# fanzhongyi/diffusion

Measured on AMD Instinct MI355X. Metric: U-Net training images/sec @256 (SD-2-base U-Net, precomputed latents 4x32x32), higher is better.
Workload: dtype bf16; 1 GPU; SD-2-base U-Net train step, latents 4x32x32, text 77x1024, batch 256/GPU (global 256), microbatch 256, AdamW, dp1; global_batch=256, microbatch=256, parallelism=dp1, params=865910724

## Files before the change

diffusion_amd/csrc/gemm_nt.hip:

```cpp
#include <string.h>

#include "common.hpp"
#include "diffusion_amd.h"

namespace {

struct GemmNTParams {
  const bf16* A;
  const bf16* W;
  void* C;
  const float* bias;
  const bf16* rowbias;
  const bf16* R;
  long lda, ldc, ldrb, ldr;
  int M, N, K, Cin;
  int Hin, Win, Hout, Wout;
  int ksize, mode;
  int out_fp32;
  float alpha;
  int tiles_m, tiles_n;
};

constexpr int BM = 128, BN = 128, BK = 64;
constexpr int STAGE_BYTES = (BM + BN) * BK * 2;
// ... 199 lines not shown

int da_gemm_nt_v2_dispatch(int variant, int splits, float* ws, const void* A, long lda, const void* W, void* C, long ldc, const float* bias,
                           const void* rowbias, long ldrb, const void* R, long ldr, int M, int N, int K, int Cin,
                           int Hin, int Win, int Hout, int Wout, int ksize, int mode, int out_fp32, float alpha,
                           hipStream_t stream);

int da_gemm_nt_v3_try(const void* A, long lda, const void* W, void* C, long ldc, const float* bias, const void* R, long ldr,
                      int M, int N, int K, hipStream_t stream);
extern int g_nt_stream, g_nt_stream_lw;
int da_gemm_nt_ws_try(const void* A, long lda, const void* W, const float* bias, const void* R, long ldr, void* C, long ldc,
                      int M, int N, int K, hipStream_t stream);
extern int g_nt_ws;

extern int g_tn_variant;
extern int g_nt_korder;
extern int g_nt_persist;
extern int g_reserve_cus;
extern int g_nt_persist_conv;
extern int g_nt_de;
extern int g_grad_overwrite;
extern int g_attn_fused_bwd;
extern int g_tn_ring, g_tn_ungroup;
extern int g_gn_resident, g_gn_resident_form, g_gn_resident_min_slab;
int da_usable_cus(int cus);
static int g_nt_variant = 0;
static int g_nt_mfma32 = 0;
static int g_nt_splitk = 1;

static int g_nt_dispatch = 1;

// ... 6 lines not shown
  if (N % 160 != 0 && tm * ((N + 127) / 128) >= 200) return 4;
  if (N % 320 == 0 && g_nt_splitk) {
    const long tiles = tm * (N / 320);
    const int nk = K / 64;
    int s = (int)((256 + tiles - 1) / tiles);
    if (s > 8) s = 8;
    while (s > 1 && (nk / s < 8 || (long)s * M * N > ws_floats)) --s;
    if (s > 1 && tiles * s >= 96) {
      *splits = s;
      return 12;
    }
  }
  return 1;
}

static int pick_nt_variant(int M, int N, int K, int Cin, long ws_floats, int* splits) {
  *splits = 1;
  if (Cin % 64 != 0) return 1;
  if (g_nt_variant == 4 || g_nt_variant == 5 || g_nt_variant == 10 || g_nt_variant == 11 || g_nt_variant == 12 || g_nt_variant == 14 ||
      g_nt_variant == 15 || g_nt_variant == 16 || g_nt_variant == 18)
    return g_nt_variant;
  if (g_nt_variant != 0) return 1;
  if (!g_nt_dispatch) return pick_nt_variant_legacy(M, N, K, Cin, ws_floats, splits);
  struct Form { int variant, bm, bn; double step_us, fixed_us; };
  static const Form forms[] = {{12, 256, 320, 1.5, 8.0}, {14, 256, 256, 1.3, 8.0}, {5, 256, 160, 1.16, 6.0}, {18, 384, 128, 1.37, 8.0},
                               {4, 256, 128, 1.07, 5.0}};
  const int nk = K / 64;
  const int ncu = da_usable_cus(256);
  double best = 1e30;
  int best_v = 4, best_s = 1;
  for (const Form& f : forms) {
    const long tiles = ((M + f.bm - 1) / f.bm) * ((N + f.bn - 1) / f.bn);
    for (int s = 1; s <= (g_nt_splitk ? 8 : 1); ++s) {
      if (s > 1 && (nk / s < 4 || (long)s * M * N > ws_floats)) break;
      const long rounds = (tiles * s + ncu - 1) / ncu;
      const int steps = (nk + s - 1) / s;
      double t = (double)rounds * (steps * f.step_us + f.fixed_us);
      if (s > 1) t += 20.0 + ((double)s * M * N * 4.0 + (double)M * N * 2.0) / 5.0e6;
      if (t < best * 0.97) {
        best = t;
        best_v = f.variant;
        best_s = s;
      }
    }
  }
  *splits = best_s;
  if (best_v == 12 && (g_nt_mfma32 == 1 || (g_nt_mfma32 < 0 && K <= 320))) return 15;
  return best_v;
}

extern "C" int da_gemm_nt_variant_for(int M, int N, int K, int Cin, long ws_floats) {
  int s;
// ... 3 lines not shown
extern "C" int da_set_option(const char* key, int value) {
  if (key && !strcmp(key, "gemm_nt_variant")) {
    g_nt_variant = value;
    return DA_OK;
  }
  if (key && !strcmp(key, "gemm_nt_splitk")) {
    g_nt_splitk = value;
    return DA_OK;
  }
  if (key && !strcmp(key, "gemm_nt_dispatch")) {
    g_nt_dispatch = value;
    return DA_OK;
  }
  if (key && !strcmp(key, "gemm_nt_persist")) {
    g_nt_persist = value;
    return DA_OK;
  }
  if (key && !strcmp(key, "gemm_nt_korder")) {
    g_nt_korder = value;
    return DA_OK;
  }
  if (key && !strcmp(key, "gemm_nt_mfma32")) {
    g_nt_mfma32 = value;
    return DA_OK;
  }
  if (key && !strcmp(key, "gemm_tn_variant")) {
    g_tn_variant = value;
    return DA_OK;
  }
  if (key && !strcmp(key, "attn_fused_bwd")) {
// ... 71 lines not shown
  if (mode == 4 && ksize != 3) return DA_ERR_SHAPE;
  if (Hout <= 0 || Wout <= 0 || (M % (Hout * Wout))) return DA_ERR_SHAPE;
  if (R && (ldr & 7)) return DA_ERR_SHAPE;
  if (rowbias && (ldrb & 7)) return DA_ERR_SHAPE;
  if (g_nt_ws && g_nt_variant == 0 && ksize == 1 && mode == 0 && !out_fp32 && alpha == 1.0f && !rowbias) {
    const int rc = da_gemm_nt_ws_try(A, lda, W, bias, R, ldr, C, ldc, M, N, K, stream);
    if (rc >= 0) return rc;
  }
  if (g_nt_stream && g_nt_variant == 0 && ksize == 1 && mode == 0 && !out_fp32 && alpha == 1.0f && !rowbias &&
      (g_nt_stream == 2 || (K <= 640 && (long)((M + 127) / 128) * ((N + 319) / 320) >= 512))) {
    const int rc = da_gemm_nt_v3_try(A, lda, W, C, ldc, bias, R, ldr, M, N, K, stream);
    if (rc >= 0) return rc;
  }
  {
    int splits = 1;
    const int variant = pick_nt_variant(M, N, K, Cin, splitk_ws ? splitk_ws_floats : 0, &splits);
    if (variant != 1)
      return da_gemm_nt_v2_dispatch(variant, splits, splitk_ws, A, lda, W, C, ldc, bias, rowbias, ldrb, R, ldr, M, N, K, Cin, Hin, Win,
                                    Hout, Wout, ksize, mode, out_fp32, alpha, stream);
  }
  GemmNTParams p;
  p.A = (const bf16*)A; p.W = (const bf16*)W; p.C = C; p.bias = bias;
  p.rowbias = (const bf16*)rowbias; p.R = (const bf16*)R;
  p.lda = lda; p.ldc = ldc; p.ldrb = ldrb; p.ldr = ldr;
  p.M = M; p.N = N; p.K = K; p.Cin = Cin;
  p.Hin = Hin; p.Win = Win; p.Hout = Hout; p.Wout = Wout;
  p.ksize = ksize; p.mode = mode; p.out_fp32 = out_fp32; p.alpha = alpha;
  p.tiles_m = (M + BM - 1) / BM;
  p.tiles_n = (N + BN - 1) / BN;
  static unsigned long long attr_done = 0;
  if (da_ensure_dyn_smem((const void*)gemm_nt_kernel, SMEM_BYTES, &attr_done) != DA_OK) return DA_ERR_LAUNCH;
// ... 5 lines not shown
```

diffusion_amd/csrc/gemm_nt_v2.hip:

```cpp
#include "common.hpp"
#include "diffusion_amd.h"
#ifndef NT2_NT
#define NT2_NT 0
#endif
#if NT2_NT
#define NTST st8_nt
#else
#define NTST st8
#endif


#ifndef NT2_CT
#define NT2_CT 1
#endif

int g_nt_persist = -1;
int g_reserve_cus = 0;
int g_nt_persist_conv = 1;
int g_nt_de = 1;
int da_usable_cus(int cus) {
  int n = cus - g_reserve_cus;
  return n < 32 ? 32 : n;
}

namespace {

struct GemmNT2Params {
  const bf16* A;
  const bf16* W;
  void* C;
  const float* bias;
  const bf16* rowbias;
  const bf16* R;
  long lda, ldc, ldrb, ldr;
  int M, N, K, Cin;
  int Hin, Win, Hout, Wout;
  int ksize, mode;
  int out_fp32;
  float alpha;
  int tiles_m, tiles_n;
  int splits, ksteps_per_split;
  long slab_stride;
  bf16* G;
  long ldg;
  int inner;
  int total_blocks;
  FastDiv div_hw, div_w;
  FastDiv div_nblk, div_tn;
  int korder;
};

__device__ __attribute__((aligned(256))) unsigned char g_zero_page[256];

template <int BK>
DEVINL int swz_key(int row) { return BK == 64 ? ((row >> 1) & 7) : ((row >> 2) & 3); }
template <int BK>
DEVINL int swz2(int row, int chunk) { return row * (BK * 2) + ((chunk ^ swz_key<BK>(row)) << 4); }

DEVINL void lds_barrier() {
  asm volatile("s_waitcnt lgkmcnt(0)" ::: "memory");
  __builtin_amdgcn_s_barrier();
  asm volatile("" ::: "memory");
}

// ... 4 lines not shown
    if (threadIdx.x == 0 && g_stamp_buf) g_stamp_buf[(long)vblock * 16 + (i)] = __builtin_amdgcn_s_memtime(); \
  } while (0)
extern "C" int da_debug_set_stamps(void* buf) {
  return hipMemcpyToSymbol(HIP_SYMBOL(g_stamp_buf), &buf, sizeof(buf)) == hipSuccess ? 0 : -1;
}
#else
#define STAMP(i) do {} while (0)
#endif

DEVINL void glds16(const void* gsrc, char* lds_dst) {
  __builtin_amdgcn_global_load_lds((const __attribute__((address_space(1))) void*)gsrc,
                                   (__attribute__((address_space(3))) void*)lds_dst, 16, 0, 0);
}

template <int MT, int NT, int WM, int WN, int BK, bool UPS, int GEGLU, bool EARLY, int MF = 16, bool PERSIST = EARLY, bool DE = false,
          bool HASR = false>
DEVINL void nt2_tile(const GemmNT2Params& p, const int vblock0, char* smem) {
  constexpr int NW = WM * WN;
  constexpr bool CT = MF == 16 && GEGLU == 0 && ((NT2_CT && !EARLY) || DE);
  static_assert(!DE || (MF == 16 && GEGLU == 0 && ((NT % 2) == 0 || (MT % 2) == 0)), "direct epilogue: 16x16 tiles in pairs");
  constexpr int V2_BM = MF * MT * WM, V2_BK = BK;
  static_assert((NW == 16 || NW == 8 || NW == 4) && (BK == 64 || BK == 32), "wave grid");
  static_assert(MF == 16 || (MF == 32 && GEGLU == 0 && BK == 64), "MFMA shape");
  constexpr int BN = MF * NT * WN;
  constexpr int SR = MF == 16 ? 16 : 8;
  constexpr int RG = 512 / BK;
  constexpr int LR = BK / 8;
  constexpr int AJ = V2_BM / RG / NW;
  constexpr int BGROUPS = BN / RG;
  constexpr int BJ = (BGROUPS + NW - 1) / NW;
  constexpr int A_BYTES = V2_BM * V2_BK * 2;
  constexpr int B_BYTES = BN * V2_BK * 2;
  constexpr int STAGE = A_BYTES + B_BYTES;
// ... 9 lines not shown
  const int wm = wave / WN, wn = wave % WN;
  auto task_of = [&](int ln, int pss, int tasks) {
    const bool ragged_last = (tasks % (64 * WN)) != 0 && pss == (tasks + 64 * WN - 1) / (64 * WN) - 1;
    const int slot = ragged_last ? (wn + WN - (wm * WN / 4) % WN) % WN : wn;
    return slot * 64 + ln + 64 * WN * pss;
  };
  auto fresh_lane = [&]() {
    int ln = lane;
    asm volatile("" : "+v"(ln));
    return ln;
  };
  STAMP(0);

  const int nblk = p.tiles_m * p.tiles_n;
  int split, tn, m0, n0;
  auto locate = [&](int vb) {
    split = (PERSIST && !EARLY) ? (int)fdiv((unsigned)vb, p.div_nblk) : vb / nblk;
    int bid = vb - split * nblk;
    const int q = nblk >> 3, r = nblk & 7;
    const int xcd = bid & 7, idx = bid >> 3;
    bid = (xcd < r ? xcd * (q + 1) : r * (q + 1) + (xcd - r) * q) + idx;
    const int tm = (PERSIST && !EARLY) ? (int)fdiv((unsigned)bid, p.div_tn) : bid / p.tiles_n;
    tn = bid - tm * p.tiles_n;
    m0 = tm * V2_BM;
    n0 = tn * BN;
  };
  auto wrow = [&](int c) {
    if constexpr (GEGLU == 1) return c < BN / 2 ? tn * (BN / 2) + c : p.inner + tn * (BN / 2) + (c - BN / 2);
    else return n0 + c;
  };
  const int HWo = p.Hout * p.Wout;
  constexpr bool PCONV = PERSIST && !EARLY;
  const int pad = PCONV ? 1 : ((p.ksize == 3 && p.mode != 4) ? 1 : 0);
  const int gmul = PCONV ? 1 : ((p.mode == 1 || p.mode == 4) ? 2 : 1), gshift = PCONV ? 0 : ((p.mode == 2 || p.mode == 3) ? 1 : 0),
            pmask = PCONV ? 0 : ((p.mode == 2) ? 1 : 0);
  const int hlim = gshift ? 2 * p.Hin : p.Hin, wlim = gshift ? 2 * p.Win : p.Win;
  const char* zero = reinterpret_cast<const char*>(g_zero_page);
  auto load_bias = [&](int buf) {
    if (tid < BN / 4) {
      const int n = wrow(tid * 4);
      const void* src = (p.bias && n < p.N) ? (const void*)(p.bias + n) : (const void*)zero;
      glds16(src, smem + BIAS_OFF + buf * (BN * 4) + wave * 1024);
    }
  };

  const int ntaps = PCONV ? 9 : p.ksize * p.ksize;
  const bf16* abase[AJ];
  unsigned amask[AJ];
  unsigned aoff[AJ];
  unsigned woff[BJ];
  int nk, tap, c0;
  const int nk_total = p.K / V2_BK;
  const bool tap_inner = p.korder != 0 && ntaps > 1;
  auto describe = [&]() {
  const int dl = fresh_lane();
  const int lrow = dl / LR, lchunk = dl % LR;
#pragma unroll
  for (int j = 0; j < AJ; ++j) {
    const int row = (wave * AJ + j) * RG + lrow;
    const int m = m0 + row;
    const bool mval = m < p.M;
    if constexpr (EARLY) {
#ifdef NT2_EXP_AHOT
      aoff[j] = (unsigned)(row) * (unsigned)(p.lda * 2) + (lchunk ^ swz_key<BK>(row)) * 16;
#else
      aoff[j] = (unsigned)(mval ? m : 0) * (unsigned)(p.lda * 2) + (lchunk ^ swz_key<BK>(row)) * 16;
#endif
      continue;
    }
    const int mm = mval ? m : 0;
    int b, rem, oh;
    if constexpr (PERSIST) {
      b = (int)fdiv((unsigned)mm, p.div_hw);
      rem = mm - b * HWo;
      oh = (int)fdiv((unsigned)rem, p.div_w);
    } else {
      b = mm / HWo;
      rem = mm - b * HWo;
      oh = rem / p.Wout;
    }
    const int ow = rem - oh * p.Wout;
    unsigned mask = ((oh & 1) << 16) | ((ow & 1) << 17);
    for (int t = 0; t < ntaps; ++t) {
      const int r = (PCONV || p.ksize == 3) ? t / 3 : 0, s2 = (PCONV || p.ksize == 3) ? t - 3 * r : 0;
      const int th = oh * gmul + r - pad, tw = ow * gmul + s2 - pad;
      const bool ok = mval && (unsigned)th < (unsigned)hlim && (unsigned)tw < (unsigned)wlim && !((th | tw) & pmask);
      mask |= (ok ? 1u : 0u) << t;
    }
    const int bh = (oh * gmul - pad) >> gshift, bw = (ow * gmul - pad) >> gshift;
    if constexpr (PERSIST && !UPS) {
      aoff[j] = (unsigned)(((long)(b * p.Hin * p.Win) + (long)bh * p.Win + bw) * p.lda * 2 + (lchunk ^ swz_key<BK>(row)) * 16);
      if (j == 0) amask[0] = mask & 0x1ffu;
      else amask[0] |= (mask & 0x1ffu) << (9 * j);
      continue;
    }
    amask[j] = mask;
    abase[j] = p.A + ((long)(b * p.Hin * p.Win) + (long)bh * p.Win + bw) * p.lda + (lchunk ^ swz_key<BK>(row)) * 8;
  }
#pragma unroll
  for (int j = 0; j < BJ; ++j) {
    const int g = wave + NW * j;
    const int row = g * RG + lrow;
    const int n = min(wrow(row), p.N - 1);
    woff[j] = ((unsigned)n * (unsigned)p.K + (lchunk ^ swz_key<BK>(row)) * 8) * 2;
  }

  const int kstep_begin = split * p.ksteps_per_split;
  nk = min(p.ksteps_per_split, nk_total - kstep_begin);
  if (tap_inner) {
    const int ch = kstep_begin / ntaps;
    tap = kstep_begin - ch * ntaps;
    c0 = ch * V2_BK;
  } else {
    const int kb = kstep_begin * V2_BK;
    tap = kb / p.Cin;
    c0 = kb - tap * p.Cin;
  }
  };
  auto issue = [&](int stage, bool live) {
    char* Ab = smem + stage * STAGE;
    char* Bb = Ab + A_BYTES;
    const int r = tap / 3, s2 = tap - 3 * r;
    const unsigned tapbit = live ? (1u << tap) : 0u;
// ... 30 lines not shown
        glds16(src, Ab + (wave * AJ + j) * 1024);
      }
    }
    const char* wb = reinterpret_cast<const char*>(p.W + (live ? tap * p.Cin + c0 : 0));
#pragma unroll
    for (int j = 0; j < BJ; ++j) {
      const int g = wave + NW * j;
      if constexpr (PERSIST && !EARLY) {
        if (BGROUPS % NW == 0 || g < BGROUPS) glds16(wb + (size_t)j * (NW * RG) * p.K * 2 + woff[0], Bb + g * 1024);
      } else {
        if (BGROUPS % NW == 0 || g < BGROUPS) glds16(wb + woff[j], Bb + g * 1024);
      }
    }
    const int tap_n = tap + 1, c_n = c0 + V2_BK;
    const bool wrap_t = tap_n >= ntaps, wrap_c = c_n >= p.Cin;
    if (tap_inner) {
      tap = wrap_t ? 0 : tap_n;
      c0 = wrap_t ? c_n : c0;
    } else {
      c0 = wrap_c ? 0 : c_n;
      tap = wrap_c ? tap_n : tap;
    }
  };

  typedef float accv_t __attribute__((ext_vector_type(MF == 16 ? 4 : 16)));
  accv_t acc[MT][NT];

  auto compute_half = [&](int stage, int s) {
    const char* Ab = smem + stage * STAGE;
    const char* Bb = Ab + A_BYTES;
    bf16x8 a[MT], b[NT];
// ... 81 lines not shown
      KSTAMP(2);
    } else {
      issue((t + 1) & 1, t + 1 < nk);
      compute_half(t & 1, 0);
    }
    __syncthreads();
    KSTAMP(3);
  }
#ifdef DA_STAMPS
  if (threadIdx.x == 0 && g_stamp_buf)
    for (int i = 0; i < 4; ++i) g_stamp_buf[(long)vblock * 16 + 8 + i] = ph[i];
#endif
  STAMP(3);
  };

  auto epilogue = [&](const int m0e, const int n0e, const int tne, const int splite, const int bbuf) {
  if constexpr (DE) {
    typedef unsigned u32x2_t __attribute__((ext_vector_type(2)));
    constexpr int NPJ = NT / 2;
    constexpr bool ODD = (NT & 1) != 0;
    constexpr int IH = ODD ? ((MT / 2 + 1) / 2) * 2 : (MT + 1) / 2;
    const int ln = fresh_lane();
    char* const cb = reinterpret_cast<char*>(p.C);
    const char* const rb = reinterpret_cast<const char*>(p.R);
    const int lrow = wm * (16 * MT) + (ln & 15), lq = (ln >> 4) & 1, lcol = wn * (16 * NT) + 8 * (ln >> 5);
    auto row_of = [&](int i) { return m0e + lrow + i * 16; };
    auto col_of = [&](int pj) { return n0e + lcol + 32 * pj + 16 * lq; };
    auto row5_of = [&](int i) { return m0e + lrow + (i - 1 + lq) * 16; };
    const int col5 = n0e + lcol + 16 * (NT - 1);
    u32x4 rin[MT][NPJ > 0 ? NPJ : 1], rin5[MT];
    auto fetch = [&](const int i_lo, const int i_hi) {
#pragma unroll
      for (int i = 0; i < MT; ++i) {
        if (i < i_lo || i >= i_hi) continue;
        const unsigned mo = (unsigned)min(row_of(i), p.M - 1) * (unsigned)(p.ldr * 2);
#pragma unroll
        for (int pj = 0; pj < NPJ; ++pj)
          rin[i][pj] = *reinterpret_cast<const u32x4*>(rb + (mo + (unsigned)min(col_of(pj), p.N - 8) * 2u));
        if constexpr (ODD) {
          if (i & 1)
            rin5[i] = *reinterpret_cast<const u32x4*>(rb + ((unsigned)min(row5_of(i), p.M - 1) * (unsigned)(p.ldr * 2) +
                                                            (unsigned)min(col5, p.N - 8) * 2u));
        }
      }
    };
    auto finish = [&](accv_t a, accv_t b, const u32x4 r, const int ma, const int mb, const int na, const int nb) {
      if (p.rowbias) {
        const int ia = (PERSIST && !EARLY) ? (int)fdiv((unsigned)min(ma, p.M - 1), p.div_hw) : min(ma, p.M - 1) / HWo;
        const int ib = (PERSIST && !EARLY) ? (int)fdiv((unsigned)min(mb, p.M - 1), p.div_hw) : min(mb, p.M - 1) / HWo;
        const bf16x4 ra = *reinterpret_cast<const bf16x4*>(p.rowbias + (long)ia * p.ldrb + min(na, p.N - 4));
        const bf16x4 rb4 = *reinterpret_cast<const bf16x4*>(p.rowbias + (long)ib * p.ldrb + min(nb, p.N - 4));
#pragma unroll
        for (int e = 0; e < 4; ++e) {
          a[e] += bf2f(ra[e]);
          b[e] += bf2f(rb4[e]);
        }
// ... 22 lines not shown
#pragma unroll
    for (int i = 0; i < MT; ++i) {
      if constexpr (HASR) {
        if (i == IH) fetch(IH, MT);
      }
      const int m = row_of(i);
      const int ma = m0e + wm * (16 * MT) + i * 16 + (ln & 15);
#pragma unroll
      for (int pj = 0; pj < NPJ; ++pj) {
        const int n = col_of(pj);
        const int na = n0e + wn * (16 * NT) + 32 * pj + aq;
        const u32x4 o = finish(acc[i][2 * pj], acc[i][2 * pj + 1], rin[i][pj], ma, ma, na, na + 16);
#ifdef NT2_EXP_NOSTORE
        asm volatile("" ::"v"(o));
#else
        if (m < p.M && n < p.N) *reinterpret_cast<u32x4*>(cb + ((unsigned)m * (unsigned)(p.ldc * 2) + (unsigned)n * 2u)) = o;
#endif
      }
      if constexpr (ODD) {
        if (i & 1) {
          const int m5 = row5_of(i);
          const int na = n0e + wn * (16 * NT) + 16 * (NT - 1) + aq;
          const u32x4 o = finish(acc[i - 1][NT - 1], acc[i][NT - 1], rin5[i], ma - 16, ma, na, na);
#ifdef NT2_EXP_NOSTORE
          asm volatile("" ::"v"(o));
#else
          if (m5 < p.M && col5 < p.N) *reinterpret_cast<u32x4*>(cb + ((unsigned)m5 * (unsigned)(p.ldc * 2) + (unsigned)col5 * 2u)) = o;
#endif
        }
      }
    }
    STAMP(4);
    return;
  }
  const float* bias_lds = reinterpret_cast<const float*>(smem + BIAS_OFF + bbuf * (BN * 4));
  float* const strips = reinterpret_cast<float*>(smem + STRIP_OFF);
  const int el = fresh_lane();
  if constexpr (GEGLU == 1) {
    static_assert(BN == 320 && !UPS, "GEGLU tile = 160 value + 160 gate columns");
    constexpr int GLD = BN + 4, GSTRIP = 16 * GLD, HC = BN / 2;
    constexpr int GTASKS = 16 * (HC / 8), GPASSES = (GTASKS + 64 * WN - 1) / (64 * WN);
    const int mrow0g = m0e + wm * (16 * MT);
// ... 113 lines not shown
  bool tval[PASSES];
#pragma unroll
  for (int pss = 0; pss < PASSES; ++pss) {
    const int task = task_of(el, pss, TASKS);
    trow[pss] = task / CH;
    tcol[pss] = (task - trow[pss] * CH) * 8;
    tval[pss] = task < TASKS && n0e + tcol[pss] < p.N;
  }
  const int mrow0 = m0e + wm * (MF * MT);
  const bool has_r = p.R != nullptr && p.splits == 1;
  bf16x8 rres[RD][PASSES];
  auto fetch_r = [&](int i, int slot) {
#pragma unroll
    for (int pss = 0; pss < PASSES; ++pss) {
      const int m = mrow0 + i * SR + trow[pss];
      if (tval[pss] && m < p.M) rres[slot][pss] = ld8(p.R + (long)m * p.ldr + n0e + tcol[pss]);
    }
  };
#pragma unroll
  for (int i = 0; i < RD; ++i) {
#pragma unroll
    for (int pss = 0; pss < PASSES; ++pss) rres[i][pss] = bf16x8{0, 0, 0, 0, 0, 0, 0, 0};
    if (has_r) fetch_r(i, i);
  }
#pragma unroll
  for (int i = 0; i < NSI; ++i) {
    float* ew = strips + ((EPI_DB ? (i & 1) * WM : 0) + wm) * STRIP;
#pragma unroll
    for (int j = 0; j < NT; ++j) {
      if constexpr (CT) {
        *reinterpret_cast<f32x4*>(&ew[(el & 15) * EPI_LD + wn * (16 * NT) + j * 16 + (el >> 4) * 4]) = acc[i][j];
      } else {
#pragma unroll
        for (int e = 0; e < 4; ++e) {
          if constexpr (MF == 16) ew[((el >> 4) * 4 + e) * EPI_LD + wn * (16 * NT) + j * 16 + (el & 15)] = acc[i][j][e];
          else ew[((el >> 5) * 4 + e) * EPI_LD + wn * (32 * NT) + j * 32 + (el & 31)] = acc[i / 4][j][(i & 3) * 4 + e];
        }
      }
    }
    lds_barrier();
#pragma unroll
    for (int pss = 0; pss < PASSES; ++pss) {
      const int row = trow[pss], col8 = tcol[pss];
      const int m = mrow0 + i * SR + row;
      const int n = n0e + col8;
      if (tval[pss] && m < p.M) {
        const f32x4 v0 = *reinterpret_cast<const f32x4*>(&ew[row * EPI_LD + col8]);
        const f32x4 v1 = *reinterpret_cast<const f32x4*>(&ew[row * EPI_LD + col8 + 4]);
        if (p.splits > 1) {
          float* cp = reinterpret_cast<float*>(p.C) + splite * p.slab_stride + (long)m * p.N + n;
          *reinterpret_cast<f32x4*>(cp) = v0;
          *reinterpret_cast<f32x4*>(cp + 4) = v1;
          continue;
        }
        float v[8];
        if (fold_bias) {
#pragma unroll
          for (int e = 0; e < 4; ++e) {
            v[e] = v0[e];
            v[e + 4] = v1[e];
          }
// ... 27 lines not shown
          for (int e = 0; e < 8; ++e) o[e] = f2bf(v[e]);
          if constexpr (EARLY) NTST(reinterpret_cast<bf16*>(p.C) + (long)m * p.ldc + n, o);
          else st8(reinterpret_cast<bf16*>(p.C) + (long)m * p.ldc + n, o);
        }
      }
    }
    if (has_r && i + RD < NSI) fetch_r(i + RD, i % RD);
    if (!EPI_DB) lds_barrier();
    STAMP(4 + i);
  }
  };

  locate(vblock);
  load_bias(0);
  describe();
  issue(0, true);
  if constexpr (!PERSIST) {
    kloop(0);
    epilogue(m0, n0, tn, split, 0);
  } else {
    for (int bbuf = 0;; bbuf ^= 1) {
      kloop(bbuf);
      const int m0e = m0, n0e = n0, tne = tn, splite = split;
      const int vnext = vblock + (int)gridDim.x;
      const bool more = vnext < p.total_blocks;
      if (more) {
        locate(vnext);
        load_bias(bbuf ^ 1);
        describe();
        issue(0, true);
      }
      STAMP(8);
      epilogue(m0e, n0e, tne, splite, bbuf);
      STAMP(12);
      if (!more) break;
      vblock = vnext;
    }
  }
}

template <int MT, int NT, int WM, int WN, int BK, bool UPS, int GEGLU = 0, bool EARLY = false, int MF = 16, bool PERSIST = EARLY, bool DE = false,
          bool HASR = false>
__global__ __launch_bounds__(64 * WM * WN, (WM * WN == 16 ? 4 : 2)) void gemm_nt2_kernel(GemmNT2Params p) {
  extern __shared__ __attribute__((aligned(16))) char smem[];
  nt2_tile<MT, NT, WM, WN, BK, UPS, GEGLU, EARLY, MF, PERSIST, DE, HASR>(p, blockIdx.x, smem);
}

__global__ void splitk_finalize_kernel(GemmNT2Params p, const float* ws) {
  const int nvec = p.N >> 3;
  const long total = (long)p.M * nvec;
  const int HWo = p.Hout * p.Wout;
  for (long i = (long)blockIdx.x * blockDim.x + threadIdx.x; i < total; i += (long)gridDim.x * blockDim.x) {
    const long m = i / nvec;
    const int n = (int)(i - m * nvec) * 8;
    float v[8] = {0.f, 0.f, 0.f, 0.f, 0.f, 0.f, 0.f, 0.f};
#pragma unroll 4
    for (int s = 0; s < p.splits; ++s) {
      const float* src = ws + s * p.slab_stride + m * p.N + n;
      const f32x4 a = *reinterpret_cast<const f32x4*>(src), b = *reinterpret_cast<const f32x4*>(src + 4);
#pragma unroll
// ... 28 lines not shown
}

static int persistent_grid(int total_blocks) {
  if (g_nt_persist == 0) return total_blocks;
  int n = g_nt_persist;
  if (n < 0) {
    static int cus[64];
    int dev = 0;
    if (hipGetDevice(&dev) != hipSuccess || dev < 0 || dev >= 64) return total_blocks;
    if (!cus[dev] && hipDeviceGetAttribute(&cus[dev], hipDeviceAttributeMultiprocessorCount, dev) != hipSuccess) cus[dev] = 256;
    n = da_usable_cus(cus[dev]);
  }
  return total_blocks < n ? total_blocks : n;
}

template <int MT, int NT, int WM, int WN, int BK, bool UPS, bool EARLY, int MF = 16, bool PERSIST = EARLY>
int launch_v2_mode(const GemmNT2Params& p0, int splits, float* ws, hipStream_t stream) {
  GemmNT2Params p = p0;
  constexpr int V2_BM = MF * MT * WM, V2_BK = BK, NTHREADS = 64 * WM * WN;
  constexpr int BN = MF * NT * WN;
  constexpr int STAGE = V2_BM * V2_BK * 2 + BN * V2_BK * 2, STRIPS = WM * (MF == 16 ? 16 : 8) * (BN + 4) * 4;
  constexpr int SMEM = PERSIST ? (STAGE + STRIPS > 2 * STAGE ? STAGE + STRIPS : 2 * STAGE) + 2 * BN * 4 : 2 * STAGE + BN * 4;
  static_assert(2 * STAGE >= STRIPS && SMEM <= 160 * 1024, "LDS map of nt2_tile");
  p.tiles_m = (p.M + V2_BM - 1) / V2_BM;
  p.tiles_n = (p.N + BN - 1) / BN;
  static unsigned long long attr_done = 0;
  if (da_ensure_dyn_smem((const void*)gemm_nt2_kernel<MT, NT, WM, WN, BK, UPS, 0, EARLY, MF, PERSIST>, SMEM, &attr_done) != DA_OK) return DA_ERR_LAUNCH;
  const int nk_total = p.K / V2_BK;
  p.splits = splits > 1 ? splits : 1;
  p.ksteps_per_split = (nk_total + p.splits - 1) / p.splits;
  p.splits = (nk_total + p.ksteps_per_split - 1) / p.ksteps_per_split;
  p.slab_stride = (long)p.M * p.N;
  p.total_blocks = p.tiles_m * p.tiles_n * p.splits;
  p.div_nblk = make_fastdiv((unsigned)(p.tiles_m * p.tiles_n));
  p.div_tn = make_fastdiv((unsigned)p.tiles_n);
  if (PERSIST && (p.total_blocks >= (1 << 20) || p.M >= (1 << 24))) return DA_ERR_SHAPE;
  const int grid = PERSIST ? persistent_grid(p.total_blocks) : p.total_blocks;
  if (p.splits > 1) {
    GemmNT2Params pk = p;
    pk.C = ws;
    hipLaunchKernelGGL((gemm_nt2_kernel<MT, NT, WM, WN, BK, UPS, 0, EARLY, MF, PERSIST>), dim3(grid), dim3(NTHREADS), SMEM,
                       stream, pk);
    DA_CHECK_LAUNCH();
    const long total = (long)p.M * (p.N >> 3);
    long blocks = (total + 255) / 256;
    if (blocks > 4096) blocks = 4096;
    hipLaunchKernelGGL(splitk_finalize_kernel, dim3((int)blocks), dim3(256), 0, stream, p, (const float*)ws);
    DA_CHECK_LAUNCH();
    return DA_OK;
  }
  if constexpr (MF == 16 && ((NT % 2) == 0 || (MT % 2) == 0)) {
    const bool form_ok = !EARLY || g_nt_de >= 3 || (g_nt_de == 2 && !p.R);
    const bool de = g_nt_de && form_ok && !p.out_fp32 && p.alpha == 1.0f && (p.N % 8) == 0 && (p.ldc % 8) == 0 && !((uintptr_t)p.C & 15) &&
                    (long)p.M * p.ldc * 2 < (1L << 32) &&
                    (!p.R || ((p.ldr % 8) == 0 && !((uintptr_t)p.R & 15) && (long)p.M * p.ldr * 2 < (1L << 32))) &&
                    (!p.rowbias || ((p.ldrb % 4) == 0 && !((uintptr_t)p.rowbias & 7)));
    if (de) {
      static unsigned long long attr_done_de[2] = {0, 0};
      if (p.R) {
        if (da_ensure_dyn_smem((const void*)gemm_nt2_kernel<MT, NT, WM, WN, BK, UPS, 0, EARLY, MF, PERSIST, true, true>, SMEM, &attr_done_de[1]) != DA_OK)
          return DA_ERR_LAUNCH;
        hipLaunchKernelGGL((gemm_nt2_kernel<MT, NT, WM, WN, BK, UPS, 0, EARLY, MF, PERSIST, true, true>), dim3(grid), dim3(NTHREADS), SMEM, stream, p);
      } else {
        if (da_ensure_dyn_smem((const void*)gemm_nt2_kernel<MT, NT, WM, WN, BK, UPS, 0, EARLY, MF, PERSIST, true, false>, SMEM, &attr_done_de[0]) != DA_OK)
          return DA_ERR_LAUNCH;
        hipLaunchKernelGGL((gemm_nt2_kernel<MT, NT, WM, WN, BK, UPS, 0, EARLY, MF, PERSIST, true, false>), dim3(grid), dim3(NTHREADS), SMEM, stream, p);
      }
      DA_CHECK_LAUNCH();
      return DA_OK;
    }
  }
  hipLaunchKernelGGL((gemm_nt2_kernel<MT, NT, WM, WN, BK, UPS, 0, EARLY, MF, PERSIST>), dim3(grid), dim3(NTHREADS), SMEM, stream, p);
  DA_CHECK_LAUNCH();
  return DA_OK;
}

template <int GM>
int launch_v2_geglu(GemmNT2Params p, hipStream_t stream) {
  constexpr int BN = 320, STAGE = 256 * 64 * 2 + BN * 64 * 2, STRIPS = 4 * 16 * (BN + 4) * 4;
  constexpr int SMEM = (STAGE + STRIPS > 2 * STAGE ? STAGE + STRIPS : 2 * STAGE) + 2 * BN * 4;
  static_assert(SMEM <= 160 * 1024, "LDS");
  p.tiles_m = (p.M + 255) / 256;
  p.tiles_n = GM == 1 ? (p.inner + BN / 2 - 1) / (BN / 2) : (p.inner + BN - 1) / BN;
  p.splits = 1;
  p.ksteps_per_split = p.K / 64;
  static unsigned long long attr_done = 0;
  if (da_ensure_dyn_smem((const void*)gemm_nt2_kernel<4, 5, 4, 4, 64, false, GM, true>, SMEM, &attr_done) != DA_OK) return DA_ERR_LAUNCH;
// ... 8 lines not shown

template <int MT, int NT, int WM, int WN, int BK, int MF = 16>
int launch_v2(const GemmNT2Params& p, int splits, float* ws, hipStream_t stream) {
  if (p.mode == 3) return launch_v2_mode<MT, NT, WM, WN, BK, true, false, MF>(p, splits, ws, stream);
  if ((long)p.N * p.K * 2 >= (1L << 32)) return DA_ERR_SHAPE;
  if constexpr (WM * WN == 16) {
    if (p.ksize == 1 && (long)p.M * p.lda * 2 < (1L << 32)) return launch_v2_mode<MT, NT, WM, WN, BK, false, true, MF>(p, splits, ws, stream);
  }
  if constexpr (WM * WN == 16 && MF == 16 && MT == 4 && NT == 5) {
    const long tiles = (long)((p.M + 255) / 256) * ((p.N + 319) / 320) * (splits > 1 ? splits : 1);
    if (g_nt_persist_conv && g_nt_persist != 0 && p.ksize == 3 && p.mode == 0 && tiles > da_usable_cus(256) && p.N % 320 == 0 &&
        p.M < (1 << 24) && (long)p.M * p.Hout * p.Wout < (1L << 40) &&
        (long)(p.M / (p.Hout * p.Wout)) * p.Hin * p.Win * p.lda * 2 < (1L << 32))
      return launch_v2_mode<MT, NT, WM, WN, BK, false, false, MF, true>(p, splits, ws, stream);
  }
  return launch_v2_mode<MT, NT, WM, WN, BK, false, false, MF>(p, splits, ws, stream);
}

}

int g_nt_korder = 1;

int da_gemm_nt_v2_dispatch(int variant, int splits, float* ws, const void* A, long lda, const void* W, void* C, long ldc, const float* bias,
                           const void* rowbias, long ldrb, const void* R, long ldr, int M, int N, int K, int Cin,
                           int Hin, int Win, int Hout, int Wout, int ksize, int mode, int out_fp32, float alpha,
                           hipStream_t stream) {
  GemmNT2Params p;
  p.A = (const bf16*)A; p.W = (const bf16*)W; p.C = C; p.bias = bias;
  p.rowbias = (const bf16*)rowbias; p.R = (const bf16*)R;
  p.lda = lda; p.ldc = ldc; p.ldrb = ldrb; p.ldr = ldr;
  p.M = M; p.N = N; p.K = K; p.Cin = Cin;
  p.Hin = Hin; p.Win = Win; p.Hout = Hout; p.Wout = Wout;
  p.ksize = ksize; p.mode = mode; p.out_fp32 = out_fp32; p.alpha = alpha;
  p.tiles_m = p.tiles_n = 0;
  p.splits = 1; p.ksteps_per_split = 0; p.slab_stride = 0;
  p.G = nullptr; p.ldg = 0; p.inner = 0;
  p.korder = g_nt_korder;
  p.total_blocks = 0;
  p.div_hw = make_fastdiv((unsigned)(Hout * Wout));
  p.div_w = make_fastdiv((unsigned)Wout);
  p.div_nblk = p.div_tn = make_fastdiv(1u);
  if (variant == 10) return launch_v2<8, 5, 2, 4, 64>(p, splits, ws, stream);
  if (variant == 11) return launch_v2<4, 10, 2, 2, 32>(p, 1, ws, stream);
  if (variant == 12) return launch_v2<4, 5, 4, 4, 64>(p, splits, ws, stream);
  if (variant == 15) return launch_v2<1, 5, 8, 2, 64, 32>(p, splits, ws, stream);
  if (variant == 16) return launch_v2<2, 5, 4, 2, 64, 32>(p, splits, ws, stream);
  if (variant == 18) return launch_v2<3, 4, 8, 2, 64>(p, splits, ws, stream);
  if (variant == 14) return launch_v2<4, 4, 4, 4, 64>(p, splits, ws, stream);
  return variant == 5 ? launch_v2<4, 5, 4, 2, 64>(p, splits, ws, stream) : launch_v2<4, 4, 4, 2, 64>(p, splits, ws, stream);
}

// ... 8 lines not shown
  if ((long)M * lda * 2 >= (1L << 32) || (long)inner * K * 4 >= (1L << 32)) return DA_ERR_SHAPE;
  {
    const int rc = da_gemm_nt_geglu_ws_try(A, lda, W, bias, F, ldf, G, ldg, M, inner, K, stream);
    if (rc >= 0) return rc;
  }
  GemmNT2Params p;
  p.A = (const bf16*)A; p.W = (const bf16*)W; p.C = F; p.bias = bias;
  p.rowbias = nullptr; p.R = nullptr;
  p.lda = lda; p.ldc = ldf; p.ldrb = 0; p.ldr = 0;
  p.M = M; p.N = 2 * inner; p.K = K; p.Cin = K;
  p.Hin = 1; p.Win = 1; p.Hout = 1; p.Wout = 1;
  p.ksize = 1; p.mode = 0; p.out_fp32 = 0; p.alpha = 1.0f;
  p.tiles_m = p.tiles_n = 0;
  p.splits = 1; p.ksteps_per_split = 0; p.slab_stride = 0;
  p.G = (bf16*)G; p.ldg = ldg; p.inner = inner; p.korder = 0; p.total_blocks = 0;
  p.div_hw = p.div_w = p.div_nblk = p.div_tn = make_fastdiv(1u);
  return launch_v2_geglu<1>(p, stream);
}

extern "C" int da_gemm_nt_geglu_bwd(const void* dY, long lddy, const void* Wt, const void* F, long ldf, void* dF, long lddf,
                                    int M, int inner, int K, hipStream_t stream) {
  DA_CLEAR_ERR();
  if (M <= 0 || inner <= 0 || K <= 0) return DA_ERR_SHAPE;
  if ((inner % 320) || (K % 64) || (lddy & 7) || (ldf & 7) || (lddf & 7)) return DA_ERR_SHAPE;
  if ((long)M * lddy * 2 >= (1L << 32) || (long)inner * K * 2 >= (1L << 32)) return DA_ERR_SHAPE;
  GemmNT2Params p;
  p.A = (const bf16*)dY; p.W = (const bf16*)Wt; p.C = dF; p.bias = nullptr;
  p.rowbias = nullptr; p.R = nullptr;
  p.lda = lddy; p.ldc = lddf; p.ldrb = 0; p.ldr = 0;
  p.M = M; p.N = inner; p.K = K; p.Cin = K;
  p.Hin = 1; p.Win = 1; p.Hout = 1; p.Wout = 1;
  p.ksize = 1; p.mode = 0; p.out_fp32 = 0; p.alpha = 1.0f;
  p.tiles_m = p.tiles_n = 0;
  p.splits = 1; p.ksteps_per_split = 0; p.slab_stride = 0;
  p.G = (bf16*)const_cast<void*>(F); p.ldg = ldf; p.inner = inner; p.korder = 0; p.total_blocks = 0;
  p.div_hw = p.div_w = p.div_nblk = p.div_tn = make_fastdiv(1u);
  return launch_v2_geglu<2>(p, stream);
}
```

Before: 1532 images/sec.

## Walk stride-2 transposed-conv dgrad by output parity class to skip zero taps

```diff
diff --git a/diffusion_amd/csrc/gemm_nt.hip b/diffusion_amd/csrc/gemm_nt.hip
--- a/diffusion_amd/csrc/gemm_nt.hip
+++ b/diffusion_amd/csrc/gemm_nt.hip
@@ -237,6 +237,8 @@
 
 extern int g_tn_variant;
 extern int g_nt_korder;
+extern int g_nt_dgrad2_ninetap;
+int da_nt_class_walk(int M, int Hin, int Win, int Hout, int Wout, int ksize, int mode, int has_rowbias);
 extern int g_nt_persist;
 extern int g_reserve_cus;
 extern int g_nt_persist_conv;
@@ -273,7 +275,40 @@
   return 1;
 }
 
-static int pick_nt_variant(int M, int N, int K, int Cin, long ws_floats, int* splits) {
+static double class_walk_us(long tiles_per_class, const double* cost , int ncu) {
+  struct Group { double t; long n; } g[32];
+  int ng = 1;
+  g[0].t = 0.0;
+  g[0].n = ncu;
+  double end = 0.0;
+  for (int c = 0; c < 4; ++c) {
+    for (long left = tiles_per_class; left > 0;) {
+      int e = 0;
+      for (int i = 1; i < ng; ++i)
+        if (g[i].t < g[e].t) e = i;
+      const long n = g[e].n < left ? g[e].n : left;
+      const double t = g[e].t + cost[c];
+      g[e].n -= n;
+      if (!g[e].n) g[e] = g[--ng];
+      int j = 0;
+      while (j < ng && g[j].t != t) ++j;
+      if (j < ng) {
+        g[j].n += n;
+      } else if (ng < 32) {
+        g[ng].t = t;
+        g[ng].n = n;
+        ++ng;
+      } else {
+        return tiles_per_class * (cost[0] + cost[1] + cost[2] + cost[3]) / ncu + cost[0];
+      }
+      left -= n;
+      end = t > end ? t : end;
+    }
+  }
+  return end;
+}
+
+static int pick_nt_variant(int M, int N, int K, int Cin, long ws_floats, int* splits, int m2 = 0) {
   *splits = 1;
   if (Cin % 64 != 0) return 1;
   if (g_nt_variant == 4 || g_nt_variant == 5 || g_nt_variant == 10 || g_nt_variant == 11 || g_nt_variant == 12 || g_nt_variant == 14 ||
@@ -284,17 +319,25 @@
   struct Form { int variant, bm, bn; double step_us, fixed_us; };
   static const Form forms[] = {{12, 256, 320, 1.5, 8.0}, {14, 256, 256, 1.3, 8.0}, {5, 256, 160, 1.16, 6.0}, {18, 384, 128, 1.37, 8.0},
                                {4, 256, 128, 1.07, 5.0}};
-  const int nk = K / 64;
+  const int nk = m2 ? 4 * (Cin / 64) : K / 64;
   const int ncu = da_usable_cus(256);
   double best = 1e30;
   int best_v = 4, best_s = 1;
+  const int s_forced = g_nt_splitk >= 2 && nk / g_nt_splitk >= 4 && (long)g_nt_splitk * M * N <= ws_floats ? g_nt_splitk : 0;
+  const int s_lo = s_forced ? s_forced : 1, s_hi = s_forced ? s_forced : g_nt_splitk == 1 ? 8 : 1;
   for (const Form& f : forms) {
     const long tiles = ((M + f.bm - 1) / f.bm) * ((N + f.bn - 1) / f.bn);
-    for (int s = 1; s <= (g_nt_splitk ? 8 : 1); ++s) {
+    for (int s = s_lo; s <= s_hi; ++s) {
       if (s > 1 && (nk / s < 4 || (long)s * M * N > ws_floats)) break;
       const long rounds = (tiles * s + ncu - 1) / ncu;
       const int steps = (nk + s - 1) / s;
       double t = (double)rounds * (steps * f.step_us + f.fixed_us);
+      if (m2) {
+        const int nch = Cin / 64;
+        const double cost[4] = {(4 * nch + s - 1) / s * f.step_us + f.fixed_us, (2 * nch + s - 1) / s * f.step_us + f.fixed_us,
+                                (2 * nch + s - 1) / s * f.step_us + f.fixed_us, (nch + s - 1) / s * f.step_us + f.fixed_us};
+        t = class_walk_us(((M / 4 + f.bm - 1) / f.bm) * ((N + f.bn - 1) / f.bn) * s, cost, ncu);
+      }
       if (s > 1) t += 20.0 + ((double)s * M * N * 4.0 + (double)M * N * 2.0) / 5.0e6;
       if (t < best * 0.97) {
         best = t;
@@ -328,6 +371,11 @@
   }
   if (key && !strcmp(key, "gemm_nt_persist")) {
     g_nt_persist = value;
+    return DA_OK;
+  }
+  if (key && !strcmp(key, "gemm_nt_dgrad2_ninetap")) {
+    if (value != 0 && value != 1) return DA_ERR_SHAPE;
+    g_nt_dgrad2_ninetap = value;
     return DA_OK;
   }
   if (key && !strcmp(key, "gemm_nt_korder")) {
@@ -429,7 +477,8 @@
   }
   {
     int splits = 1;
-    const int variant = pick_nt_variant(M, N, K, Cin, splitk_ws ? splitk_ws_floats : 0, &splits);
+    const int variant = pick_nt_variant(M, N, K, Cin, splitk_ws ? splitk_ws_floats : 0, &splits,
+                                        da_nt_class_walk(M, Hin, Win, Hout, Wout, ksize, mode, rowbias != nullptr));
     if (variant != 1)
       return da_gemm_nt_v2_dispatch(variant, splits, splitk_ws, A, lda, W, C, ldc, bias, rowbias, ldrb, R, ldr, M, N, K, Cin, Hin, Win,
                                     Hout, Wout, ksize, mode, out_fp32, alpha, stream);
diff --git a/diffusion_amd/csrc/gemm_nt_v2.hip b/diffusion_amd/csrc/gemm_nt_v2.hip
--- a/diffusion_amd/csrc/gemm_nt_v2.hip
+++ b/diffusion_amd/csrc/gemm_nt_v2.hip
@@ -18,6 +18,12 @@
 int g_reserve_cus = 0;
 int g_nt_persist_conv = 1;
 int g_nt_de = 1;
+int g_nt_dgrad2_ninetap = 0;
+int g_nt_korder = 1;
+int da_nt_class_walk(int M, int Hin, int Win, int Hout, int Wout, int ksize, int mode, int has_rowbias) {
+  return mode == 2 && ksize == 3 && !g_nt_dgrad2_ninetap && g_nt_korder != 0 && !has_rowbias && Hout == 2 * Hin && Wout == 2 * Win &&
+         M < (1 << 24) && (long)(M / 4) * Hin * Win < (1L << 40);
+}
 int da_usable_cus(int cus) {
   int n = cus - g_reserve_cus;
   return n < 32 ? 32 : n;
@@ -48,6 +54,8 @@
   FastDiv div_hw, div_w;
   FastDiv div_nblk, div_tn;
   int korder;
+  int Mc;
+  FastDiv div_chw, div_cw;
 };
 
 __device__ __attribute__((aligned(256))) unsigned char g_zero_page[256];
@@ -82,9 +90,10 @@
 }
 
 template <int MT, int NT, int WM, int WN, int BK, bool UPS, int GEGLU, bool EARLY, int MF = 16, bool PERSIST = EARLY, bool DE = false,
-          bool HASR = false>
+          bool HASR = false, bool PC = false>
 DEVINL void nt2_tile(const GemmNT2Params& p, const int vblock0, char* smem) {
   constexpr int NW = WM * WN;
+  static_assert(!PC || (!UPS && GEGLU == 0 && !EARLY && !PERSIST && MF == 16 && BK == 64), "parity-class walk: generic 3x3 gather form");
   constexpr bool CT = MF == 16 && GEGLU == 0 && ((NT2_CT && !EARLY) || DE);
   static_assert(!DE || (MF == 16 && GEGLU == 0 && ((NT % 2) == 0 || (MT % 2) == 0)), "direct epilogue: 16x16 tiles in pairs");
   constexpr int V2_BM = MF * MT * WM, V2_BK = BK;
@@ -124,7 +133,23 @@
 
   const int nblk = p.tiles_m * p.tiles_n;
   int split, tn, m0, n0;
+  int pcls = 0;
   auto locate = [&](int vb) {
+    if constexpr (PC) {
+      split = vb / nblk;
+      const int w = vb - split * nblk, nbc = nblk >> 2;
+      const int rank = w / nbc;
+      int bid = w - rank * nbc;
+      const int q = nbc >> 3, r = nbc & 7;
+      const int xcd = bid & 7, idx = bid >> 3;
+      bid = (xcd < r ? xcd * (q + 1) : r * (q + 1) + (xcd - r) * q) + idx;
+      const int tm = bid / p.tiles_n;
+      tn = bid - tm * p.tiles_n;
+      pcls = 3 - rank;
+      m0 = tm * V2_BM;
+      n0 = tn * BN;
+      return;
+    }
     split = (PERSIST && !EARLY) ? (int)fdiv((unsigned)vb, p.div_nblk) : vb / nblk;
     int bid = vb - split * nblk;
     const int q = nblk >> 3, r = nblk & 7;
@@ -141,9 +166,9 @@
   };
   const int HWo = p.Hout * p.Wout;
   constexpr bool PCONV = PERSIST && !EARLY;
-  const int pad = PCONV ? 1 : ((p.ksize == 3 && p.mode != 4) ? 1 : 0);
-  const int gmul = PCONV ? 1 : ((p.mode == 1 || p.mode == 4) ? 2 : 1), gshift = PCONV ? 0 : ((p.mode == 2 || p.mode == 3) ? 1 : 0),
-            pmask = PCONV ? 0 : ((p.mode == 2) ? 1 : 0);
+  const int pad = (PCONV || PC) ? 1 : ((p.ksize == 3 && p.mode != 4) ? 1 : 0);
+  const int gmul = (PCONV || PC) ? 1 : ((p.mode == 1 || p.mode == 4) ? 2 : 1),
+            gshift = PC ? 1 : PCONV ? 0 : ((p.mode == 2 || p.mode == 3) ? 1 : 0), pmask = PC ? 1 : PCONV ? 0 : ((p.mode == 2) ? 1 : 0);
   const int hlim = gshift ? 2 * p.Hin : p.Hin, wlim = gshift ? 2 * p.Win : p.Win;
   const char* zero = reinterpret_cast<const char*>(g_zero_page);
   auto load_bias = [&](int buf) {
@@ -154,7 +179,7 @@
     }
   };
 
-  const int ntaps = PCONV ? 9 : p.ksize * p.ksize;
+  const int ntaps = (PCONV || PC) ? 9 : p.ksize * p.ksize;
   const bf16* abase[AJ];
   unsigned amask[AJ];
   unsigned aoff[AJ];
@@ -169,7 +194,7 @@
   for (int j = 0; j < AJ; ++j) {
     const int row = (wave * AJ + j) * RG + lrow;
     const int m = m0 + row;
-    const bool mval = m < p.M;
+    const bool mval = m < (PC ? p.Mc : p.M);
     if constexpr (EARLY) {
 #ifdef NT2_EXP_AHOT
       aoff[j] = (unsigned)(row) * (unsigned)(p.lda * 2) + (lchunk ^ swz_key<BK>(row)) * 16;
@@ -179,20 +204,27 @@
       continue;
     }
     const int mm = mval ? m : 0;
-    int b, rem, oh;
-    if constexpr (PERSIST) {
+    int b, rem, oh, ow;
+    if constexpr (PC) {
+      b = mm / (p.Hin * p.Win);
+      rem = mm - b * (p.Hin * p.Win);
+      const int i2 = rem / p.Win;
+      oh = 2 * i2 + (pcls >> 1);
+      ow = 2 * (rem - i2 * p.Win) + (pcls & 1);
+    } else if constexpr (PERSIST) {
       b = (int)fdiv((unsigned)mm, p.div_hw);
       rem = mm - b * HWo;
       oh = (int)fdiv((unsigned)rem, p.div_w);
+      ow = rem - oh * p.Wout;
     } else {
       b = mm / HWo;
       rem = mm - b * HWo;
       oh = rem / p.Wout;
-    }
-    const int ow = rem - oh * p.Wout;
+      ow = rem - oh * p.Wout;
+    }
     unsigned mask = ((oh & 1) << 16) | ((ow & 1) << 17);
     for (int t = 0; t < ntaps; ++t) {
-      const int r = (PCONV || p.ksize == 3) ? t / 3 : 0, s2 = (PCONV || p.ksize == 3) ? t - 3 * r : 0;
+      const int r = (PCONV || PC || p.ksize == 3) ? t / 3 : 0, s2 = (PCONV || PC || p.ksize == 3) ? t - 3 * r : 0;
       const int th = oh * gmul + r - pad, tw = ow * gmul + s2 - pad;
       const bool ok = mval && (unsigned)th < (unsigned)hlim && (unsigned)tw < (unsigned)wlim && !((th | tw) & pmask);
       mask |= (ok ? 1u : 0u) << t;
@@ -217,6 +249,21 @@
 
   const int kstep_begin = split * p.ksteps_per_split;
   nk = min(p.ksteps_per_split, nk_total - kstep_begin);
+  if constexpr (PC) {
+    const unsigned cb = (pcls & 1) ? 5u : 2u;
+    const unsigned tmask = (pcls & 2) ? (cb | (cb << 6)) : (cb << 3);
+    const int ntc = __builtin_popcount(tmask);
+    auto before = [&](int x) {
+      const int ch = x / 9;
+      return ch * ntc + __builtin_popcount(tmask & ((1u << (x - ch * 9)) - 1u));
+    };
+    const int ch = kstep_begin / 9, t0 = kstep_begin - ch * 9;
+    const unsigned rest = tmask >> t0;
+    nk = before(kstep_begin + nk) - before(kstep_begin);
+    tap = rest ? t0 + __builtin_ctz(rest) : __builtin_ctz(tmask);
+    c0 = (rest ? ch : ch + 1) * V2_BK;
+    return;
+  }
   if (tap_inner) {
     const int ch = kstep_begin / ntaps;
     tap = kstep_begin - ch * ntaps;
@@ -277,7 +324,12 @@
     }
     const int tap_n = tap + 1, c_n = c0 + V2_BK;
     const bool wrap_t = tap_n >= ntaps, wrap_c = c_n >= p.Cin;
-    if (tap_inner) {
+    if constexpr (PC) {
+      const int pa = pcls >> 1, pb = pcls & 1;
+      const bool last_s = !pb || s2 == 2, last_t = last_s && (!pa || r == 2);
+      tap = last_t ? (pa ? 0 : 3) + (pb ? 0 : 1) : (last_s ? tap + (pb ? 4 : 6) : tap + 2);
+      c0 = last_t ? c_n : c0;
+    } else if (tap_inner) {
       tap = wrap_t ? 0 : tap_n;
       c0 = wrap_t ? c_n : c0;
     } else {
@@ -389,6 +441,21 @@
   STAMP(3);
   };
 
+  const int mlim = PC ? p.Mc : p.M;
+  auto prow = [&](int mv) {
+    if constexpr (PC) {
+      const int bi = (int)fdiv((unsigned)mv, p.div_chw);
+      const int rem = mv - bi * (p.Hin * p.Win);
+      const int i2 = (int)fdiv((unsigned)rem, p.div_cw);
+      return bi * HWo + (2 * i2 + (pcls >> 1)) * p.Wout + 2 * (rem - i2 * p.Win) + (pcls & 1);
+    } else {
+      return mv;
+    }
+  };
+  auto srow = [&](int mv) {
+    if constexpr (PC) return prow(min(mv, mlim - 1));
+    else return mv;
+  };
   auto epilogue = [&](const int m0e, const int n0e, const int tne, const int splite, const int bbuf) {
   if constexpr (DE) {
     typedef unsigned u32x2_t __attribute__((ext_vector_type(2)));
@@ -408,13 +475,13 @@
 #pragma unroll
       for (int i = 0; i < MT; ++i) {
         if (i < i_lo || i >= i_hi) continue;
-        const unsigned mo = (unsigned)min(row_of(i), p.M - 1) * (unsigned)(p.ldr * 2);
+        const unsigned mo = (unsigned)prow(min(row_of(i), mlim - 1)) * (unsigned)(p.ldr * 2);
 #pragma unroll
         for (int pj = 0; pj < NPJ; ++pj)
           rin[i][pj] = *reinterpret_cast<const u32x4*>(rb + (mo + (unsigned)min(col_of(pj), p.N - 8) * 2u));
         if constexpr (ODD) {
           if (i & 1)
-            rin5[i] = *reinterpret_cast<const u32x4*>(rb + ((unsigned)min(row5_of(i), p.M - 1) * (unsigned)(p.ldr * 2) +
+            rin5[i] = *reinterpret_cast<const u32x4*>(rb + ((unsigned)prow(min(row5_of(i), mlim - 1)) * (unsigned)(p.ldr * 2) +
                                                             (unsigned)min(col5, p.N - 8) * 2u));
         }
       }
@@ -467,7 +534,7 @@
 #ifdef NT2_EXP_NOSTORE
         asm volatile("" ::"v"(o));
 #else
-        if (m < p.M && n < p.N) *reinterpret_cast<u32x4*>(cb + ((unsigned)m * (unsigned)(p.ldc * 2) + (unsigned)n * 2u)) = o;
+        if (m < mlim && n < p.N) *reinterpret_cast<u32x4*>(cb + ((unsigned)srow(m) * (unsigned)(p.ldc * 2) + (unsigned)n * 2u)) = o;
 #endif
       }
       if constexpr (ODD) {
@@ -478,7 +545,8 @@
 #ifdef NT2_EXP_NOSTORE
           asm volatile("" ::"v"(o));
 #else
-          if (m5 < p.M && col5 < p.N) *reinterpret_cast<u32x4*>(cb + ((unsigned)m5 * (unsigned)(p.ldc * 2) + (unsigned)col5 * 2u)) = o;
+          if (m5 < mlim && col5 < p.N)
+            *reinterpret_cast<u32x4*>(cb + ((unsigned)srow(m5) * (unsigned)(p.ldc * 2) + (unsigned)col5 * 2u)) = o;
 #endif
         }
       }
@@ -622,7 +690,7 @@
 #pragma unroll
     for (int pss = 0; pss < PASSES; ++pss) {
       const int m = mrow0 + i * SR + trow[pss];
-      if (tval[pss] && m < p.M) rres[slot][pss] = ld8(p.R + (long)m * p.ldr + n0e + tcol[pss]);
+      if (tval[pss] && m < mlim) rres[slot][pss] = ld8(p.R + (long)prow(m) * p.ldr + n0e + tcol[pss]);
     }
   };
 #pragma unroll
@@ -650,9 +718,10 @@
 #pragma unroll
     for (int pss = 0; pss < PASSES; ++pss) {
       const int row = trow[pss], col8 = tcol[pss];
-      const int m = mrow0 + i * SR + row;
+      const int mv = mrow0 + i * SR + row;
       const int n = n0e + col8;
-      if (tval[pss] && m < p.M) {
+      if (tval[pss] && mv < mlim) {
+        const int m = prow(mv);
         const f32x4 v0 = *reinterpret_cast<const f32x4*>(&ew[row * EPI_LD + col8]);
         const f32x4 v1 = *reinterpret_cast<const f32x4*>(&ew[row * EPI_LD + col8 + 4]);
         if (p.splits > 1) {
@@ -710,7 +779,7 @@
   locate(vblock);
   load_bias(0);
   describe();
-  issue(0, true);
+  issue(0, PC ? nk > 0 : true);
   if constexpr (!PERSIST) {
     kloop(0);
     epilogue(m0, n0, tn, split, 0);
@@ -736,10 +805,10 @@
 }
 
 template <int MT, int NT, int WM, int WN, int BK, bool UPS, int GEGLU = 0, bool EARLY = false, int MF = 16, bool PERSIST = EARLY, bool DE = false,
-          bool HASR = false>
+          bool HASR = false, bool PC = false>
 __global__ __launch_bounds__(64 * WM * WN, (WM * WN == 16 ? 4 : 2)) void gemm_nt2_kernel(GemmNT2Params p) {
   extern __shared__ __attribute__((aligned(16))) char smem[];
-  nt2_tile<MT, NT, WM, WN, BK, UPS, GEGLU, EARLY, MF, PERSIST, DE, HASR>(p, blockIdx.x, smem);
+  nt2_tile<MT, NT, WM, WN, BK, UPS, GEGLU, EARLY, MF, PERSIST, DE, HASR, PC>(p, blockIdx.x, smem);
 }
 
 __global__ void splitk_finalize_kernel(GemmNT2Params p, const float* ws) {
@@ -798,7 +867,7 @@
   return total_blocks < n ? total_blocks : n;
 }
 
-template <int MT, int NT, int WM, int WN, int BK, bool UPS, bool EARLY, int MF = 16, bool PERSIST = EARLY>
+template <int MT, int NT, int WM, int WN, int BK, bool UPS, bool EARLY, int MF = 16, bool PERSIST = EARLY, bool PC = false>
 int launch_v2_mode(const GemmNT2Params& p0, int splits, float* ws, hipStream_t stream) {
   GemmNT2Params p = p0;
   constexpr int V2_BM = MF * MT * WM, V2_BK = BK, NTHREADS = 64 * WM * WN;
@@ -808,8 +877,14 @@
   static_assert(2 * STAGE >= STRIPS && SMEM <= 160 * 1024, "LDS map of nt2_tile");
   p.tiles_m = (p.M + V2_BM - 1) / V2_BM;
   p.tiles_n = (p.N + BN - 1) / BN;
+  if constexpr (PC) {
+    p.Mc = p.M / 4;
+    p.tiles_m = 4 * ((p.Mc + V2_BM - 1) / V2_BM);
+    p.div_chw = make_fastdiv((unsigned)(p.Hin * p.Win));
+    p.div_cw = make_fastdiv((unsigned)p.Win);
+  }
   static unsigned long long attr_done = 0;
-  if (da_ensure_dyn_smem((const void*)gemm_nt2_kernel<MT, NT, WM, WN, BK, UPS, 0, EARLY, MF, PERSIST>, SMEM, &attr_done) != DA_OK) return DA_ERR_LAUNCH;
+  if (da_ensure_dyn_smem((const void*)gemm_nt2_kernel<MT, NT, WM, WN, BK, UPS, 0, EARLY, MF, PERSIST, false, false, PC>, SMEM, &attr_done) != DA_OK) return DA_ERR_LAUNCH;
   const int nk_total = p.K / V2_BK;
   p.splits = splits > 1 ? splits : 1;
   p.ksteps_per_split = (nk_total + p.splits - 1) / p.splits;
@@ -823,7 +898,7 @@
   if (p.splits > 1) {
     GemmNT2Params pk = p;
     pk.C = ws;
-    hipLaunchKernelGGL((gemm_nt2_kernel<MT, NT, WM, WN, BK, UPS, 0, EARLY, MF, PERSIST>), dim3(grid), dim3(NTHREADS), SMEM,
+    hipLaunchKernelGGL((gemm_nt2_kernel<MT, NT, WM, WN, BK, UPS, 0, EARLY, MF, PERSIST, false, false, PC>), dim3(grid), dim3(NTHREADS), SMEM,
                        stream, pk);
     DA_CHECK_LAUNCH();
     const long total = (long)p.M * (p.N >> 3);
@@ -842,19 +917,19 @@
     if (de) {
       static unsigned long long attr_done_de[2] = {0, 0};
       if (p.R) {
-        if (da_ensure_dyn_smem((const void*)gemm_nt2_kernel<MT, NT, WM, WN, BK, UPS, 0, EARLY, MF, PERSIST, true, true>, SMEM, &attr_done_de[1]) != DA_OK)
+        if (da_ensure_dyn_smem((const void*)gemm_nt2_kernel<MT, NT, WM, WN, BK, UPS, 0, EARLY, MF, PERSIST, true, true, PC>, SMEM, &attr_done_de[1]) != DA_OK)
           return DA_ERR_LAUNCH;
-        hipLaunchKernelGGL((gemm_nt2_kernel<MT, NT, WM, WN, BK, UPS, 0, EARLY, MF, PERSIST, true, true>), dim3(grid), dim3(NTHREADS), SMEM, stream, p);
+        hipLaunchKernelGGL((gemm_nt2_kernel<MT, NT, WM, WN, BK, UPS, 0, EARLY, MF, PERSIST, true, true, PC>), dim3(grid), dim3(NTHREADS), SMEM, stream, p);
       } else {
-        if (da_ensure_dyn_smem((const void*)gemm_nt2_kernel<MT, NT, WM, WN, BK, UPS, 0, EARLY, MF, PERSIST, true, false>, SMEM, &attr_done_de[0]) != DA_OK)
+        if (da_ensure_dyn_smem((const void*)gemm_nt2_kernel<MT, NT, WM, WN, BK, UPS, 0, EARLY, MF, PERSIST, true, false, PC>, SMEM, &attr_done_de[0]) != DA_OK)
           return DA_ERR_LAUNCH;
-        hipLaunchKernelGGL((gemm_nt2_kernel<MT, NT, WM, WN, BK, UPS, 0, EARLY, MF, PERSIST, true, false>), dim3(grid), dim3(NTHREADS), SMEM, stream, p);
+        hipLaunchKernelGGL((gemm_nt2_kernel<MT, NT, WM, WN, BK, UPS, 0, EARLY, MF, PERSIST, true, false, PC>), dim3(grid), dim3(NTHREADS), SMEM, stream, p);
       }
       DA_CHECK_LAUNCH();
       return DA_OK;
     }
   }
-  hipLaunchKernelGGL((gemm_nt2_kernel<MT, NT, WM, WN, BK, UPS, 0, EARLY, MF, PERSIST>), dim3(grid), dim3(NTHREADS), SMEM, stream, p);
+  hipLaunchKernelGGL((gemm_nt2_kernel<MT, NT, WM, WN, BK, UPS, 0, EARLY, MF, PERSIST, false, false, PC>), dim3(grid), dim3(NTHREADS), SMEM, stream, p);
   DA_CHECK_LAUNCH();
   return DA_OK;
 }
@@ -893,12 +968,14 @@
         (long)(p.M / (p.Hout * p.Wout)) * p.Hin * p.Win * p.lda * 2 < (1L << 32))
       return launch_v2_mode<MT, NT, WM, WN, BK, false, false, MF, true>(p, splits, ws, stream);
   }
+  if constexpr (MF == 16 && BK == 64) {
+    if (da_nt_class_walk(p.M, p.Hin, p.Win, p.Hout, p.Wout, p.ksize, p.mode, p.rowbias != nullptr))
+      return launch_v2_mode<MT, NT, WM, WN, BK, false, false, MF, false, true>(p, splits, ws, stream);
+  }
   return launch_v2_mode<MT, NT, WM, WN, BK, false, false, MF>(p, splits, ws, stream);
 }
 
 }
-
-int g_nt_korder = 1;
 
 int da_gemm_nt_v2_dispatch(int variant, int splits, float* ws, const void* A, long lda, const void* W, void* C, long ldc, const float* bias,
                            const void* rowbias, long ldrb, const void* R, long ldr, int M, int N, int K, int Cin,
@@ -914,6 +991,7 @@
   p.tiles_m = p.tiles_n = 0;
   p.splits = 1; p.ksteps_per_split = 0; p.slab_stride = 0;
   p.G = nullptr; p.ldg = 0; p.inner = 0;
+  p.Mc = 0; p.div_chw = p.div_cw = make_fastdiv(1u);
   p.korder = g_nt_korder;
   p.total_blocks = 0;
   p.div_hw = make_fastdiv((unsigned)(Hout * Wout));
@@ -952,7 +1030,8 @@
   p.tiles_m = p.tiles_n = 0;
   p.splits = 1; p.ksteps_per_split = 0; p.slab_stride = 0;
   p.G = (bf16*)G; p.ldg = ldg; p.inner = inner; p.korder = 0; p.total_blocks = 0;
-  p.div_hw = p.div_w = p.div_nblk = p.div_tn = make_fastdiv(1u);
+  p.Mc = 0;
+  p.div_hw = p.div_w = p.div_nblk = p.div_tn = p.div_chw = p.div_cw = make_fastdiv(1u);
   return launch_v2_geglu<1>(p, stream);
 }
 
@@ -972,6 +1051,7 @@
   p.tiles_m = p.tiles_n = 0;
   p.splits = 1; p.ksteps_per_split = 0; p.slab_stride = 0;
   p.G = (bf16*)const_cast<void*>(F); p.ldg = ldf; p.inner = inner; p.korder = 0; p.total_blocks = 0;
-  p.div_hw = p.div_w = p.div_nblk = p.div_tn = make_fastdiv(1u);
+  p.Mc = 0;
+  p.div_hw = p.div_w = p.div_nblk = p.div_tn = p.div_chw = p.div_cw = make_fastdiv(1u);
   return launch_v2_geglu<2>(p, stream);
 }
```

New measurement: 1538 images/sec, median of 6. No clear change (+0.4%).
